# warwick-hpsc/MG-CFD-app-plain

Measured on AMD Instinct MI355X. Metric: Medges/s (compute_flux_edge) + MG V-cycle wall-s, higher is better.
Workload: dtype f64; 1 GPU; M6-L0-like synthetic level (67^3 jittered lattice, permuted ids): 300763 nodes / 888822 internal edges per GPU, flux + update sweep, no MG; numerics=exact (bit-identical to the reference), parallelism=1 GPU, workload_kind=level0

## Files before the change

### include/mgcfd.h

```cpp
#ifndef MGCFD_H
#define MGCFD_H

#include <stdint.h>

#ifdef __cplusplus
extern "C" {
#endif

#define MGCFD_NVAR 5
#define MGCFD_RK 3

#define MGCFD_MESH_FVCORR 0
#define MGCFD_MESH_M6_WING 2
#define MGCFD_MESH_LA_CASCADE 3
#define MGCFD_MESH_ROTOR_37 4

#define MGCFD_OK 0
#define MGCFD_ERR_ARG 1
#define MGCFD_ERR_IO 2
#define MGCFD_ERR_HIP 3
#define MGCFD_ERR_NAN 4
#define MGCFD_ERR_NEG_DENSITY 5
#define MGCFD_ERR_NEG_ENERGY 6
#define MGCFD_ERR_VALIDATION 7
// ... 52 lines not shown
int mgcfd_mesh_level(const mgcfd_mesh *m, int level, mgcfd_level_desc *out);

int mgcfd_write_array(const char *path, const double *data, int64_t nel, int ncols);
int mgcfd_identify_differences(const double *test_values, const double *master_values, int64_t nel,
                               int mesh_variant, int64_t *first_bad);

int mgcfd_create(const mgcfd_level_desc *levels, int nlevels, int mesh_variant, int device,
                 mgcfd_solver **out);
int mgcfd_create_from_mesh(const mgcfd_mesh *m, int device, mgcfd_solver **out);
int mgcfd_create_partitioned(const mgcfd_level_desc *levels, int nlevels, int mesh_variant, int device,
                             const int64_t *n_owned, mgcfd_solver **out);
int mgcfd_create_partitioned_mg(const mgcfd_level_desc *levels, int nlevels, int mesh_variant, int device,
                                const int64_t *n_owned, const int64_t *const *order_keys, mgcfd_solver **out);
int mgcfd_plan_audit(const mgcfd_level_desc *levels, int nlevels, int mesh_variant, const int64_t *n_owned,
                     const int64_t *const *order_keys, char *report, int64_t report_cap);
void mgcfd_destroy(mgcfd_solver *s);
int mgcfd_set_option(mgcfd_solver *s, int option, int value);
int mgcfd_level_has_edge_once(const mgcfd_solver *s, int level, int *yes);
int mgcfd_level_has_half_rows(const mgcfd_solver *s, int level, int *yes);
int mgcfd_level_has_order_free(const mgcfd_solver *s, int level, int *yes);
int mgcfd_level_stage_wg4(const mgcfd_solver *s, int level, int *yes);
int mgcfd_level_tiling(const mgcfd_solver *s, int level, int64_t out[10]);
int mgcfd_get_option(const mgcfd_solver *s, int option, int *value);
int mgcfd_set_stream(mgcfd_solver *s, void *hip_stream);
int mgcfd_synchronize(mgcfd_solver *s);
int mgcfd_num_levels(const mgcfd_solver *s);
int64_t mgcfd_level_nel(const mgcfd_solver *s, int level);
int64_t mgcfd_level_num_internal_edges(const mgcfd_solver *s, int level);
int mgcfd_get_far_field(const mgcfd_solver *s, double *out17);
int mgcfd_free_stream_constants(double mach, double alpha_deg, double out17[17]);
// ... 124 lines not shown
```

### mg-cfd-app-plain_amd/csrc/device_plan.hpp

```cpp
#pragma once

#include <hip/hip_runtime.h>
#include <cstdint>

#include "preprocess.hpp"

namespace mgcfd {

constexpr int kNumStateFields = 5;
static_assert(sizeof(EdgeW) == 32, "EdgeW must be 32 bytes");
static_assert(sizeof(ProlongW) == 24, "ProlongW must be 24 bytes");

constexpr int kVariantStageWg4 = 1 << 7;

struct FarField {
    double var[5];
    double fc_mx[3], fc_my[3], fc_mz[3], fc_de[3];
};

constexpr int kMaxPushPeers = 8;
struct PushPeers {
    double *base[kMaxPushPeers] = {nullptr, nullptr, nullptr, nullptr, nullptr, nullptr, nullptr, nullptr};
    int64_t stride[kMaxPushPeers] = {0, 0, 0, 0, 0, 0, 0, 0};
    int64_t first[kMaxPushPeers + 1] = {0, 0, 0, 0, 0, 0, 0, 0, 0};
    int n = 0;
};

struct PushFlags {
// ... 113 lines not shown
    double p_inf = 0.0;
    const double *ref = nullptr;
    const int32_t *slot = nullptr;
    double *table = nullptr;
    int64_t row = 0;
};

struct TailPlan {
    const int32_t *rows_main = nullptr;
    const int32_t *tile_ptr = nullptr;
    const double2 *rec = nullptr;
    const int32_t *begin = nullptr, *count = nullptr;
    double2 *flux = nullptr;
};

struct DevicePlan {
    int64_t nel = 0;
    int64_t stride = 0;
    int32_t n_slices = 0;
    int32_t *slice_row0 = nullptr, *rows_int = nullptr, *rows_bnd = nullptr, *nbr = nullptr;
    double *w = nullptr;
    int32_t n_tiles = 0;
    int32_t pad_row = 0;
    int32_t pad_chunk = 0;
    uint16_t *nbr16 = nullptr;
    int32_t *tile_halo = nullptr;
    int32_t *tile_ovf_ptr = nullptr, *tile_ovf = nullptr;
    int vin_ok = 0;
    int lds_complete = 0;
    int32_t halo_max = 0;
    int edge_once = 0;
    int32_t *te_chunk_ptr = nullptr, *te_count = nullptr;
    uint16_t *te_slots = nullptr, *gat16 = nullptr;
    double *te_w = nullptr;
    double *te_w3 = nullptr;
// ... 31 lines not shown
```

### mg-cfd-app-plain_amd/csrc/kernels.hip

```cpp
#include <hip/hip_runtime.h>
#include <algorithm>
#include <cstdlib>
#include <stdexcept>
#include <stdint.h>
#include <type_traits>

#include "device_plan.hpp"

#ifndef MGCFD_KERNEL_NS
#error "compile with -DMGCFD_KERNEL_NS=exact|fast"
#endif

namespace mgcfd {
namespace MGCFD_KERNEL_NS {

#ifdef MGCFD_PHASES
__device__ unsigned long long g_phase[4096 * 8];
__device__ unsigned long long g_phase_abs[4096 * 8];
#define PH_MARK(k) do { if (threadIdx.x == 0) { unsigned long long now_ = wall_clock64(); g_phase[(blockIdx.x & 4095) * 8 + (k)] += now_ - ph_last_; ph_last_ = now_; g_phase_abs[(blockIdx.x & 4095) * 8 + 1 + (k)] = now_; } } while (0)
#define PH_BEGIN() unsigned long long ph_last_ = wall_clock64(); if (threadIdx.x == 0) { g_phase[(blockIdx.x & 4095) * 8 + 7] += 1ull; g_phase_abs[(blockIdx.x & 4095) * 8] = ph_last_; \
        g_phase_abs[(blockIdx.x & 4095) * 8 + 7] = (static_cast<unsigned long long>(__builtin_amdgcn_s_getreg(20 | (0 << 6) | (31 << 11))) << 32) | __builtin_amdgcn_s_getreg(4 | (0 << 6) | (31 << 11)); }
#else
#define PH_MARK(k) do { } while (0)
#define PH_BEGIN() do { } while (0)
#endif

#if defined(MGCFD_EXP_FLUX_ST_NT)
#define MGCFD_ST_FLUX(p, v) __builtin_nontemporal_store((v), (p))
#elif defined(MGCFD_EXP_FLUX_ST_PLAIN)
#define MGCFD_ST_FLUX(p, v) (*(p) = (v))
#else
#define MGCFD_ST_FLUX(p, v) __hip_atomic_store((p), (v), __ATOMIC_RELAXED, __HIP_MEMORY_SCOPE_AGENT)
#endif
#if defined(MGCFD_EXP_STAGE_ST_PLAIN)
#define MGCFD_ST_STAGE(p, v) (*(p) = (v))
#elif defined(MGCFD_EXP_STAGE_ST_NT)
#define MGCFD_ST_STAGE(p, v) __builtin_nontemporal_store((v), (p))
#else
#define MGCFD_ST_STAGE(p, v) __hip_atomic_store((p), (v), __ATOMIC_RELAXED, __HIP_MEMORY_SCOPE_AGENT)
// ... 159 lines not shown

__device__ __forceinline__ double wave_sum(double v)
{
    for (int off = 32; off > 0; off >>= 1) v += __shfl_xor(v, off);
    return v;
}

__device__ __forceinline__ unsigned long long err_key(int check, int32_t original_id, int code)
{
    return (static_cast<unsigned long long>(check) << 40) | (static_cast<unsigned long long>(uint32_t(original_id)) << 8) | unsigned(code);
}

__device__ __forceinline__ unsigned xcd_contiguous_block(unsigned b, unsigned nb)
{
    const unsigned q = nb >> 3, r = nb & 7u, x = b & 7u, k = b >> 3;
    return (x < r ? x * (q + 1) : r * (q + 1) + (x - r) * q) + k;
}

}

__global__ void __launch_bounds__(kBlock)
k_init_variables(int64_t stride, FarField ff, double *__restrict__ q)
{
    const int64_t i = blockIdx.x * int64_t(kBlock) + threadIdx.x;
    if (i >= stride) return;
    store_conserved(q, stride, i, ff.var[0], ff.var[1], ff.var[2], ff.var[3], ff.var[4]);
}

__global__ void __launch_bounds__(kBlock)
k_step_factor_local(int64_t nel, int64_t stride, const double *__restrict__ q, const double *__restrict__ cbrt_vol,
                    double cfl, double *__restrict__ step_factors, double *__restrict__ partial_min,
// ... 293 lines not shown
}

struct FluxTileLds {
    double2 tile[kTileCap * kLdsRecD2];
    double s_pm[kBlock / 64];
    double s_next[2][kBlock / 64];
};
struct FluxTileLds4 {
    double2 tile[kTileCap4 * kLdsRec80D2];
    double s_pm[kBlock / 64];
    double s_next[2][kBlock / 64];
};
static_assert(sizeof(FluxTileLds4) <= 160 * 1024 / 4, "four workgroups per CU");
static_assert(kTileCap4 - kTile < kBlock, "one halo id per thread");

template <int WMODE, bool FUSE, bool ACC, int ROLE, bool TAIL, bool PUSH, bool SLIM = false, typename Lds = FluxTileLds>
__device__ __forceinline__ void
flux_tile_body(Lds &lds, const unsigned block,
               const double *__restrict__ q, const int32_t *__restrict__ tile_halo, uint32_t n_tiles, int32_t pad_row,
               int64_t stride, int64_t nel, const int32_t *__restrict__ slice_row0,
               const int32_t *__restrict__ rows_int, const int32_t *__restrict__ rows_bnd,
               const uint16_t *__restrict__ nbr16, const double *__restrict__ w,
               const int32_t *__restrict__ tile_ovf_ptr, const int32_t *__restrict__ tile_ovf, const FarField &ff,
               double *__restrict__ fluxes, int classes, const FusedStep &fs, const TailPlan &tp,
               const uint16_t *__restrict__ gat16, const int32_t *__restrict__ te_chunk_ptr, const double *__restrict__ te_w3,
               const StagePush &push ,
               const bool block_is_tile = false )
{
    constexpr bool LOADK = WMODE == 1;
    static_assert(!PUSH || FUSE, "only a fused stage sends its message");
    PH_BEGIN();
    constexpr bool IDXW = WMODE == 2;
    static_assert(!(IDXW && TAIL), "indexed weights: levels without long rows only");
    static_assert(!SLIM || (!TAIL && !IDXW && !PUSH && ROLE != 5), "80-byte records: the stages without long rows, indexed weights, message or absorbed stage");
    double2 *const tile = lds.tile;

    double min_dt = 0.0;
    constexpr int kPartPre = 6;
    double *const s_pm = lds.s_pm;
    double pmv[kPartPre];

    const int tid = threadIdx.x;
    const int lane = tid & 63;
    unsigned t = block_is_tile ? block : xcd_contiguous_block(block, n_tiles);
    if (PUSH) {
        const unsigned nb = unsigned(push.n_boundary);
        t = block < nb ? block : nb + xcd_contiguous_block(block - nb, n_tiles - nb);
    }
    if (FUSE && fs.tile_list) t = unsigned(fs.tile_list[t]);
    const int64_t base = int64_t(t) * kTile;
    const int64_t i = base + tid;
    const int32_t slice = __builtin_amdgcn_readfirstlane(static_cast<int32_t>(i >> 6));

    const int32_t *hrow = tile_halo + int64_t(t) * kHaloStride;
    const int32_t hid = hrow[tid];
    const int32_t hid2 = (!SLIM && ROLE != 5 && tid < kHaloStride - kBlock) ? hrow[kBlock + tid] : -1;
    const int32_t row0 = slice_row0[slice];
    const int32_t n_int = (classes & 1) ? (TAIL ? tp.rows_main : rows_int)[slice] : 0;
    const int32_t n_bnd = rows_bnd[slice];
    const bool has_halo = hid >= 0;
    const int64_t hnode = has_halo ? int64_t(hid) : i;
    double o0, o1, o2, o3, o4, g0, g1, g2, g3, g4;
    EdgeRow e0, e1;
    RowRef i0{}, i1{}, i2{}, i3{};
    const double *tw = nullptr;
    if (IDXW) {
        i0 = load_ref(nbr16, gat16, n_int > 0 ? row0 : pad_row, lane);
        i1 = load_ref(nbr16, gat16, n_int > 1 ? row0 + 1 : pad_row, lane);
        i2 = load_ref(nbr16, gat16, n_int > 2 ? row0 + 2 : pad_row, lane);
        i3 = load_ref(nbr16, gat16, n_int > 3 ? row0 + 3 : pad_row, lane);
        tw = te_w3 + int64_t(te_chunk_ptr[t]) * (kEdgeChunk * 3);
    }
    if (FUSE && ROLE == 5) {
#pragma unroll
// ... 229 lines not shown
            }                                                                                                     \
        } while (0)
        if (n_glob > 0) {
            const double2 *in = tp.flux + 3 * int64_t(tl_nb);
            MGCFD_ADD_ENTRIES(in, n_glob);
        }
        {
            const double2 *in = tile + 3 * (tl_nb + n_glob - last0);
            const int32_t n_lds = tl_nc - n_glob;
            MGCFD_ADD_ENTRIES(in, n_lds);
        }
#undef MGCFD_ADD_ENTRIES
    }

    if ((classes & 6) && n_bnd > 0) {
        const int32_t first_bnd = rows_int[slice];
        const FluxC fm = fm_pre;
        for (int32_t r = 0; r < n_bnd; r++) {
            const EdgeRow e = load_row<false>(nbr16, w, int64_t(row0) + first_bnd + r, lane);
            const double fx = e.fx, fy = e.fy, fz = e.fz;
            if (e.code == kT16Wall && (classes & 2)) {
                a0 += 0.0;
                a1 += fx * me.p;
                a2 += fy * me.p;
                a3 += fz * me.p;
                a4 += 0.0;
            } else if (e.code == kT16Far && (classes & 4)) {
                a0 += fx * (ff.var[1] + me.mx) + fy * (ff.var[2] + me.my) + fz * (ff.var[3] + me.mz);
                a4 += fx * (ff.fc_de[0] + fm.ex) + fy * (ff.fc_de[1] + fm.ey) + fz * (ff.fc_de[2] + fm.ez);
                a1 += fx * (ff.fc_mx[0] + fm.xx) + fy * (ff.fc_mx[1] + fm.xy) + fz * (ff.fc_mx[2] + fm.xz);
                a2 += fx * (ff.fc_my[0] + fm.xy) + fy * (ff.fc_my[1] + fm.yy) + fz * (ff.fc_my[2] + fm.yz);
                a3 += fx * (ff.fc_mz[0] + fm.xz) + fy * (ff.fc_mz[1] + fm.yz) + fz * (ff.fc_mz[2] + fm.zz);
            }
        }
// ... 9 lines not shown
    }
    double sf_next = __longlong_as_double(0x7FF0000000000000LL);
    double ss = 0.0;
    if (i < nel) {
        double sf = sfv;
        if (ROLE == 0 || ROLE == 5) {
            min_dt = s_pm[0];
            for (int wv = 1; wv < kBlock / 64; wv++) min_dt = fmin(min_dt, s_pm[wv]);
            sf = min_dt / sfv;
            fs.step_factors[i] = sf;
        }
        const double factor = sf / fs.rk_div;
        const double rho = r0 + factor * a0, mx = r1 + factor * a1, my = r2 + factor * a2, mz = r3 + factor * a3,
                     en = r4 + factor * a4;
        store_conserved(fs.q_out, stride, i, rho, mx, my, mz, en);
        if (ROLE >= 2 && ROLE <= 4) {
            const double d0 = rho - r0, d1 = mx - r1, d2 = my - r2, d3 = mz - r3, d4 = en - r4;
            if (fs.residuals) {
                MGCFD_ST_STAGE(fs.residuals + i, d0); MGCFD_ST_STAGE(fs.residuals + stride + i, d1); MGCFD_ST_STAGE(fs.residuals + 2 * stride + i, d2);
                MGCFD_ST_STAGE(fs.residuals + 3 * stride + i, d3); MGCFD_ST_STAGE(fs.residuals + 4 * stride + i, d4);
            }
            if (fs.sumsq_partial) ss = (((d0 * d0 + d1 * d1) + d2 * d2) + d3 * d3) + d4 * d4;
        }
        if (fs.check) {
            const bool finite = isfinite(rho) && isfinite(mx) && isfinite(my) && isfinite(mz) && isfinite(en);
            int code = 0;
            if (!finite) code = 1;
            else if (rho < 0.0) code = 2;
            else if (en < 0.0) code = 3;
            if (code) atomicMin(fs.err, err_key(fs.check, fs.old_of_new[i], code));
// ... 38 lines not shown
        double (*const s_next)[kBlock / 64] = lds.s_next;
        if (ROLE == 3) sf_next = wave_min(sf_next);
        if (fs.sumsq_partial) ss = wave_sum(ss);
        if ((threadIdx.x & 63) == 0) { s_next[0][threadIdx.x >> 6] = sf_next; s_next[1][threadIdx.x >> 6] = ss; }
        __syncthreads();
        if (threadIdx.x == 0) {
            double m = s_next[0][0], sum = s_next[1][0];
            for (int wv = 1; wv < kBlock / 64; wv++) { m = fmin(m, s_next[0][wv]); sum += s_next[1][wv]; }
            if (ROLE == 3) fs.next_partial_min[t] = m;
            if (fs.sumsq_partial) fs.sumsq_partial[t] = sum;
        }
    }
    PH_MARK(3);
}

template <int MINW, int WMODE, bool FUSE, bool ACC, int ROLE, bool TAIL, bool PUSH = false, bool SLIM = false>
__global__ void __launch_bounds__(kBlock, MINW)
k_flux_tile(
            const double *__restrict__ q, const int32_t *__restrict__ tile_halo, uint32_t n_tiles, int32_t pad_row,
            int64_t stride, int64_t nel, const int32_t *__restrict__ slice_row0,
            const int32_t *__restrict__ rows_int, const int32_t *__restrict__ rows_bnd,
            const uint16_t *__restrict__ nbr16, const double *__restrict__ w,
            const int32_t *__restrict__ tile_ovf_ptr, const int32_t *__restrict__ tile_ovf, FarField ff,
            double *__restrict__ fluxes, int classes, FusedStep fs, TailPlan tp,
            const uint16_t *__restrict__ gat16, const int32_t *__restrict__ te_chunk_ptr, const double *__restrict__ te_w3,
            StagePush push)
{
    __shared__ std::conditional_t<SLIM, FluxTileLds4, FluxTileLds> lds;
    flux_tile_body<WMODE, FUSE, ACC, ROLE, TAIL, PUSH, SLIM>(lds, blockIdx.x, q, tile_halo, n_tiles, pad_row, stride, nel, slice_row0, rows_int, rows_bnd, nbr16, w,
                                                       tile_ovf_ptr, tile_ovf, ff, fluxes, classes, fs, tp, gat16, te_chunk_ptr, te_w3, push);
}

struct TileEdge { uint32_t sa, sb; double fx, fy, fz, k; };
constexpr int kGatherPre = 8;

template <bool LOADK>
__device__ __forceinline__ TileEdge load_tile_edge(const uint16_t *__restrict__ te_slots, const double *__restrict__ te_w,
                                                   int64_t chunk, int tid)
{
    TileEdge e;
    e.sa = te_slots[(chunk * 2) * kEdgeChunk + tid];
    e.sb = te_slots[(chunk * 2 + 1) * kEdgeChunk + tid];
    const double *wr = te_w + chunk * (4 * kEdgeChunk) + tid;
    e.fx = wr[0]; e.fy = wr[kEdgeChunk]; e.fz = wr[2 * kEdgeChunk];
    e.k = LOADK ? wr[3 * kEdgeChunk] : 0.0;
// ... 403 lines not shown
    double min_dt = 0.0;
    if (FUSE && !SPEC && fs.partial_min) min_dt = block_min_of_partials(fs.partial_min, fs.n_partial);
    constexpr int kPartPre = 6;
    __shared__ double s_pm[kBlock / 64];
    double pmv[kPartPre];

    const int tid = threadIdx.x;
    const int lane = tid & 63;
    const unsigned t = xcd_contiguous_block(blockIdx.x, n_tiles);
    const int64_t i = int64_t(t) * kTile + tid;
    const int32_t slice = __builtin_amdgcn_readfirstlane(static_cast<int32_t>(i >> 6));

    const int32_t *hrow = tile_halo + int64_t(t) * (WIDE ? kFreeHaloStride : kHaloStride);
    const int32_t hid = hrow[tid];
    const int32_t hid2 = (WIDE || tid < kHaloStride - kBlock) ? hrow[kBlock + tid] : -1;
    const int32_t h0 = hr_row0[slice];
    const int32_t n_h = (classes & 1) ? hr_row0[slice + 1] - h0 : 0;
    const int32_t n_bnd = rows_bnd[slice];
#ifdef MGCFD_ABL_FREE_OWN_AOS
    const double2 oa_ = *reinterpret_cast<const double2 *>(q + 5 * i), ob_ = *reinterpret_cast<const double2 *>(q + 5 * i + 2);
    const double o0 = oa_.x, o1 = oa_.y, o2 = ob_.x, o3 = ob_.y, o4 = q[5 * i + 4];
#else
    const double o0 = MGCFD_LD_STATE(q + i), o1 = MGCFD_LD_STATE(q + stride + i), o2 = MGCFD_LD_STATE(q + 2 * stride + i),
                 o3 = MGCFD_LD_STATE(q + 3 * stride + i), o4 = MGCFD_LD_STATE(q + 4 * stride + i);
#endif
    EdgeRow er[kHalfMaxRows];
#ifdef MGCFD_EXP_FREE_ORDER
    constexpr int kRowsFirst = MGCFD_EXP_FREE_ORDER;
#else
    constexpr int kRowsFirst = 2;
#endif
#pragma unroll
    for (int j = 0; j < kRowsFirst; j++) er[j] = load_half_row(hr_code, hr_w, j < n_h ? h0 + j : hr_pad_row, lane);
    const int64_t hnode = hid >= 0 ? int64_t(hid) : i;
#if defined(MGCFD_ABL_FREE_HALO) && MGCFD_ABL_FREE_HALO == 1
    const double2 ga_ = *reinterpret_cast<const double2 *>(q + 5 * hnode), gb_ = *reinterpret_cast<const double2 *>(q + 5 * hnode + 2);
    const double g0 = ga_.x, g1 = ga_.y, g2 = gb_.x, g3 = gb_.y, g4 = q[5 * hnode + 4];
#elif defined(MGCFD_ABL_FREE_HALO) && MGCFD_ABL_FREE_HALO == 2
    const double2 ga_ = *reinterpret_cast<const double2 *>(q + 8 * (hnode >> 1)), gb_ = *reinterpret_cast<const double2 *>(q + 8 * (hnode >> 1) + 2);
    const double g0 = ga_.x, g1 = ga_.y, g2 = gb_.x, g3 = gb_.y, g4 = q[8 * (hnode >> 1) + 4];
// ... 1507 lines not shown
template <typename F>
static void with_bool(bool b, F &&f) { if (b) f(std::true_type{}); else f(std::false_type{}); }
template <typename F>
static void with_kind(bool fused, bool accumulate, F &&f)
{
    if (fused) f(std::true_type{}, std::false_type{});
    else if (accumulate) f(std::false_type{}, std::true_type{});
    else f(std::false_type{}, std::false_type{});
}

struct FluxLaunch {
    hipStream_t st; const DevicePlan &p; const double *q; const FarField &ff; double *fluxes; int classes; const FusedStep &fs;
    dim3 grid; int64_t nel_arg;
};

template <int WMODE, bool FUSE, bool ACC, int ROLE, bool TAIL, bool PUSH = false, bool SLIM = false>
static void launch_tile(const FluxLaunch &a, const StagePush &push = StagePush{})
{
    const DevicePlan &p = a.p;
    constexpr int MINW = SLIM ? 4 : ((TAIL && (ACC || ROLE == 5)) ? 2 : 3);
    hipLaunchKernelGGL((k_flux_tile<MINW, WMODE, FUSE, ACC, ROLE, TAIL, PUSH, SLIM>), a.grid, dim3(kBlock), 0, a.st, a.q, p.tile_halo,
                       uint32_t(a.grid.x), p.pad_row, p.stride, a.nel_arg, p.slice_row0, p.rows_int, p.rows_bnd,
                       p.nbr16, p.w, p.tile_ovf_ptr, p.tile_ovf, a.ff, a.fluxes, a.classes, a.fs, p.tail, p.gat16,
                       p.te_chunk_ptr, p.te_w3, push);
}

#ifdef MGCFD_ORDER_FREE
template <bool FUSE, bool ACC, int CAP, bool LONG, bool WIDE = false, int ROLE = -1>
static void launch_free(const FluxLaunch &a)
{
    const DevicePlan &p = a.p;
    hipLaunchKernelGGL((k_flux_free<FUSE, ACC, CAP, LONG, WIDE, ROLE>), a.grid, dim3(kBlock), 0, a.st, a.q, WIDE ? p.free_halo : p.tile_halo, uint32_t(p.n_tiles),
                       p.hr_pad_row, p.stride, p.nel, p.hr_row0, p.hr_code, p.hr_w, p.slice_row0,
                       p.rows_int, p.rows_bnd, p.nbr16, p.w, a.ff, a.fluxes, a.classes, a.fs);
}

static int free_stage_role(const FusedStep &fs, int role)
{
    if (fs.next_legacy_sf) return -1;
// ... 19 lines not shown

void launch_flux(hipStream_t st, const DevicePlan &p, const double *q, const FarField &ff, double *fluxes,
                 int classes, int accumulate, int variant, const FusedStep *fused, const StagePush *push)
{
    FusedStep fs{};
    if (fused) fs = *fused;
    const bool part = fused && fs.tile_list;
    if (part && fs.n_list <= 0) return;
    const FluxLaunch a{st, p, q, ff, fluxes, classes, fs, dim3(part ? fs.n_list : p.n_tiles), (fused && fs.nel_active > 0) ? fs.nel_active : p.nel};
    const int role = fused ? stage_role(fs) : 1;
    const bool tail = p.has_tail && (classes & 1);
    const bool loadk = (variant & 1) == 0;
    if (push && fused && part && !fs.vin_flux) {
        check_first_stage_input(role, q, fs);
        with_bool(loadk, [&](auto K) { with_bool(tail, [&](auto T) { with_constant<0, 1, 2, 3, 4>(role, [&](auto R) {
            launch_tile<decltype(K)::value ? 1 : 0, true, false, decltype(R)::value, decltype(T)::value, true>(a, *push);
        }); }); });
        return;
    }
    check_first_stage_input(role, q, fs);
    if ((variant & 4) && !fused && p.edge_flux) {
        if (classes & 1)
            hipLaunchKernelGGL(k_fission_edge_flux, dim3(grid_for(p.n_edges)), dim3(kBlock), 0, st, p.n_edges, p.n_edges_pad, p.stride, q,
                               p.fe_ab, p.fe_w, p.edge_flux);
        with_bool(accumulate != 0, [&](auto A) {
            hipLaunchKernelGGL(k_fission_node_sum<decltype(A)::value>, a.grid, dim3(kBlock), 0, st, p.nel, p.stride, p.n_edges_pad, q, p.slice_row0,
                               p.rows_int, p.rows_bnd, p.row_edge, p.nbr16, p.w, p.edge_flux, ff, fluxes, classes);
        });
        return;
    }
#ifdef MGCFD_ORDER_FREE
// ... 21 lines not shown
            hipLaunchKernelGGL((k_flux_half<decltype(F)::value, decltype(A)::value>), a.grid, dim3(kBlock), 0, st, q, p.tile_halo, uint32_t(p.n_tiles),
                               p.hr_pad_row, p.stride, p.nel, p.hr_row0, p.hr_code, p.hr_w, p.hg16, p.slice_row0,
                               p.rows_int, p.rows_bnd, p.pad_row, p.nbr16, p.w, ff, fluxes, classes, fs);
        });
        return;
    }
    if ((variant & 2) && p.edge_once && (classes & 1) && !part) {
        with_bool(loadk, [&](auto K) { with_kind(fused, accumulate, [&](auto F, auto A) {
            hipLaunchKernelGGL((k_flux_edge_once<decltype(K)::value, decltype(F)::value, decltype(A)::value>), a.grid, dim3(kBlock), 0, st, q, p.tile_halo,
                               uint32_t(p.n_tiles), p.pad_row, p.stride, p.nel, p.te_chunk_ptr, p.te_count,
                               p.pad_chunk, classes, p.slice_row0, p.rows_int, p.rows_bnd, p.nbr16, p.w, p.gat16,
                               p.te_slots, p.te_w, p.tile_ovf_ptr, p.tile_ovf, ff, fluxes, fs);
        }); });
        return;
    }
    const bool indexed = (variant & 16) && p.edge_once && p.te_w3 && !tail;
#ifndef MGCFD_ORDER_FREE
    if (fused && (variant & kVariantStageWg4) && stage_wg4_fits(p) && !indexed && role != 5) {
        with_bool(loadk, [&](auto K) { with_constant<0, 1, 2, 3, 4>(role, [&](auto R) {
            launch_tile<decltype(K)::value ? 1 : 0, true, false, decltype(R)::value, false, false, true>(a);
        }); });
        return;
    }
#endif
    with_constant<0, 1, 2>(indexed ? 2 : (loadk ? 1 : 0), [&](auto W) { with_bool(tail, [&](auto T) {
        constexpr int WMODE = decltype(W)::value;
        constexpr bool TAIL = decltype(T)::value;
        if constexpr (!(WMODE == 2 && TAIL)) {
            if (fused) with_constant<0, 1, 2, 3, 4, 5>(role, [&](auto R) { launch_tile<WMODE, true, false, decltype(R)::value, TAIL>(a); });
            else if (accumulate) launch_tile<WMODE, false, true, 1, TAIL>(a);
            else launch_tile<WMODE, false, false, 1, TAIL>(a);
        }
    }); });
}

__global__ void __launch_bounds__(kBlock)
k_stream_tiles(const double2 *__restrict__ src, double *__restrict__ dst, int64_t rd_total2, int64_t wr_total, int rd2_per_thread, int wr_per_thread)
{
    __shared__ double lds[40960 / 8 - 64];
    const int64_t r0 = int64_t(blockIdx.x) * rd2_per_thread * kBlock + threadIdx.x;
    double acc = 0.0;
    for (int k = 0; k < rd2_per_thread; k += 8) {
        double2 v[8];
#pragma unroll
// ... 241 lines not shown
```

### mg-cfd-app-plain_amd/csrc/solver.cpp

```cpp
#include <hip/hip_runtime.h>
#include <dlfcn.h>

#include <functional>
#include <future>

#include <algorithm>
#include <atomic>
#include <cmath>
#include <cstdio>
#include <cstdlib>
#include <chrono>
#include <cstring>
#include <limits>
#include <map>
#include <memory>
#include <mutex>
#include <optional>
#include <stdexcept>
#include <string>
#include <thread>
#include <vector>

#include "device_owner.hpp"
#include "kernels.hpp"
// ... 443 lines not shown
    bool stage_wg4_for(const DeviceLevel &lv) const
    {
        if (!opt_exact || !opt_stage_wg4 || !stage_wg4_fits(lv.dp)) return false;
        if (n_cus == 0) {
            use_device();
            HIP_CHECK(hipDeviceGetAttribute(&n_cus, hipDeviceAttributeMultiprocessorCount, device));
        }
        return lv.dp.n_tiles > 3 * n_cus;
    }
    void op_flux(int l, int classes)
    {
        DeviceLevel &lv = level(l);
        Timed t(this, l, MGCFD_LOOP_FLUX, (classes & 1) != 0);
        if (classes != 7) settle_fluxes(lv);
        const int accumulate = lv.fluxes_zero ? 0 : 1;
        const int variant = variant_for(lv);
        if ((variant & 4) && !lv.dp.edge_flux)
            lv.dp.edge_flux = lv.mem.alloc<double>(static_cast<size_t>(lv.dp.n_edges_pad) * 5 + 8);
        k().flux(stream, lv.dp, lv.q, ff, lv.fluxes, classes, accumulate, variant, nullptr, nullptr);
        if ((classes & 1) && jst_on(l)) {
            const JstStep a = jst_step(lv);
            k().jst_sensor(stream, lv.dp, a);
            k().jst_dissipation(stream, lv.dp, a);
        }
        if (dual_time()) lv.flux_in = lv.q;
        lv.fluxes_zero = false;
        lv.fluxes_stale = false;
        if (classes & 1) lv.iters[MGCFD_LOOP_FLUX] += lv.info.n_internal;
    }
    void op_fused_stage(int l, int j, const double *in, double *out, const StageArgs &a = StageArgs{})
    {
// ... 393 lines not shown
        st.alloc(lv.residuals, sizeof(double) * (static_cast<size_t>(stride) * 5));
        st.alloc(lv.step_factors, sizeof(double) * (static_cast<size_t>(stride)));
        st.alloc(lv.sf_alt, sizeof(double) * (static_cast<size_t>(stride)));
        st.alloc(lv.min_dt, sizeof(double) * (1));
        st.upload(lv.partial_min, std::vector<double>(static_cast<size_t>((nel + 255) / 256), std::numeric_limits<double>::infinity()));
        st.alloc(lv.tile_sumsq, sizeof(double) * (static_cast<size_t>((nel + 255) / 256)));
        st.alloc(lv.sumsq, sizeof(double) * (1));
        lv.n_partials = static_cast<int>(std::min<int64_t>(1024, (nel * 5 + 255) / 256));
        st.alloc(lv.partials, sizeof(double) * (static_cast<size_t>(lv.n_partials)));
        lv.dp.nel = nel;
        lv.dp.stride = stride;
        lv.dp.n_slices = P.n_slices;
        st.upload(lv.dp.slice_row0, P.slice_row0);
        st.upload(lv.dp.rows_int, P.rows_int);
        st.upload(lv.dp.rows_bnd, P.rows_bnd);
        {
            std::vector<double> ws(P.w.size() * 4 + 2 * 4 * kSlice, 0.0);
            for (size_t e = 0; e < P.w.size(); e++) {
                const size_t row = e / kSlice, lane = e % kSlice;
                ws[(row * 4 + 0) * kSlice + lane] = P.w[e].x;
                ws[(row * 4 + 1) * kSlice + lane] = P.w[e].y;
                ws[(row * 4 + 2) * kSlice + lane] = P.w[e].z;
                ws[(row * 4 + 3) * kSlice + lane] = P.w[e].k;
            }
            st.upload(lv.dp.w, std::move(ws));
        }
        st.upload(lv.dp.old_of_new, P.old_of_new);
        lv.dp.n_tiles = P.n_tiles;
        lv.plan.nbr16.resize(P.nbr16.size() + 2 * kSlice, static_cast<uint16_t>(kT16Pad));
        st.upload(lv.dp.nbr16, P.nbr16);
// ... 258 lines not shown
        }
        for (int l = 0; l < nlevels; l++) {
            const std::string r = audit_level_plan(levels[l], plans[static_cast<size_t>(l)], l + 1 < nlevels ? levels[l + 1].nel : -1);
            if (!r.empty()) rep += "level " + std::to_string(l) + ":\n" + r;
            if (std::getenv("MGCFD_PLAN_DIGEST")) {
                char buf[64];
                std::snprintf(buf, sizeof(buf), "digest level %d: %016llx\n", l, (unsigned long long)plan_digest(plans[static_cast<size_t>(l)]));
                rep += buf;
            }
        }
    });
    if (rc != MGCFD_OK) return rc;
    if (report && report_cap > 0) { std::snprintf(report, static_cast<size_t>(report_cap), "%s", rep.c_str()); }
    if (!rep.empty()) { g_last_error = "plan audit: " + rep; return MGCFD_ERR_ARG; }
    return MGCFD_OK;
}

int mgcfd_create(const mgcfd_level_desc *levels, int nlevels, int mesh_variant, int device, mgcfd_solver **out)
{
    REQUIRE(out);
    return guarded([&] { *out = build_solver(levels, nlevels, mesh_variant, device).release(); });
}
int mgcfd_create_partitioned(const mgcfd_level_desc *levels, int nlevels, int mesh_variant, int device,
                             const int64_t *n_owned, mgcfd_solver **out)
{
    REQUIRE(out); REQUIRE(n_owned);
    return guarded([&] { *out = build_solver(levels, nlevels, mesh_variant, device, n_owned).release(); });
}
int mgcfd_create_partitioned_mg(const mgcfd_level_desc *levels, int nlevels, int mesh_variant, int device,
                                const int64_t *n_owned, const int64_t *const *order_keys, mgcfd_solver **out)
// ... 1089 lines not shown
        s->use_device();
        s->fold_events();
        DeviceLevel &lv = s->level(level);
        *launches = lv.flux_launches;
        *avg_seconds = lv.flux_launches ? lv.flux_time / double(lv.flux_launches) : 0.0;
    });
}

int mgcfd_bench_flux(mgcfd_solver *s, int level, int launches, double *avg_seconds)
{
    REQUIRE(s); REQUIRE(avg_seconds);
    return guarded([&] {
        s->use_device();
        DeviceLevel &lv = s->level(level);
        Event a = s->get_event(), b = s->get_event();
        const int variant = s->variant_for(lv);
        if ((variant & 4) && !lv.dp.edge_flux)
            lv.dp.edge_flux = lv.mem.alloc<double>(static_cast<size_t>(lv.dp.n_edges_pad) * 5 + 8);
        auto go = [&] {
            s->k().flux(s->stream, lv.dp, lv.q, s->ff, lv.fluxes, 7, 0, variant, nullptr, nullptr);
        };
        go();
        HIP_CHECK(hipEventRecord(a.get(), s->stream));
        for (int k = 0; k < launches; k++) go();
        HIP_CHECK(hipEventRecord(b.get(), s->stream));
        HIP_CHECK(hipStreamSynchronize(s->stream));
        float ms = 0.f;
        HIP_CHECK(hipEventElapsedTime(&ms, a.get(), b.get()));
        s->free_events.push_back(std::move(a));
        s->free_events.push_back(std::move(b));
        lv.fluxes_zero = false;
// ... 2206 lines not shown
```

### mg-cfd-app-plain_amd/mgcfd/__init__.py

```python
from . import meshgen
from .api import (EXPORTED_SYMBOLS, LIB_PATH, LOOPS, Group, MgcfdError, Mesh, Solver,
                  free_stream_constants, generated_to_levels, live_device_resources, load_coefficients, load_library, plan_audit,
                  rccl_unique_id)
```

### mg-cfd-app-plain_amd/mgcfd/api.py

```python
from __future__ import annotations

import ctypes as C
import os
import sys
from typing import List, Optional, Sequence

import numpy as np

from .meshgen import EDGE_DTYPE, LevelMesh, MultigridMesh, to_edge_arrays

PKG_DIR = os.path.dirname(os.path.abspath(__file__))
CSRC_DIR = os.path.normpath(os.path.join(PKG_DIR, "..", "csrc"))
LIB_PATH = os.environ.get("MGCFD_LIB") or os.path.join(CSRC_DIR, "libmgcfd_hip.so")

NVAR = 5
RK = 3
LOOPS = ("flux", "update", "compute_step", "time_step", "restrict", "prolong", "indirect_rw")
ARR = {"variables": 0, "old_variables": 1, "fluxes": 2, "residuals": 3, "step_factors": 4, "volumes": 5, "stage": 6,
       "time_n": 7, "time_n1": 8, "jst_laplacian": 9, "jst_sensor": 10, "jst_radius": 11,
       "fas_forcing": 12, "fas_start": 13}
OPT = {"exact": 0, "timing": 1, "indirect_rw": 2, "check_invalid": 3, "flux_variant": 4, "fuse_update": 5, "graph": 6, "rank_split": 7, "stage_wg4": 8}
ERR_NAMES = {0: "OK", 1: "ERR_ARG", 2: "ERR_IO", 3: "ERR_HIP", 4: "ERR_NAN", 5: "ERR_NEG_DENSITY",
             6: "ERR_NEG_ENERGY", 7: "ERR_VALIDATION"}

# ... 27 lines not shown

_SIGNATURES = [
    ("mgcfd_last_error", C.c_char_p, []),
    ("mgcfd_abi_version", C.c_int, []),
    ("mgcfd_mesh_load", C.c_int, [C.c_char_p, C.c_char_p, C.c_int, C.POINTER(_vp)]),
    ("mgcfd_mesh_load_ex", C.c_int, [C.c_char_p, C.c_char_p, C.c_int, C.c_int, C.POINTER(_vp)]),
    ("mgcfd_mesh_free", None, [_vp]),
    ("mgcfd_mesh_num_levels", C.c_int, [_vp]),
    ("mgcfd_mesh_variant", C.c_int, [_vp]),
    ("mgcfd_mesh_size", C.c_int, [_vp]),
    ("mgcfd_mesh_level", C.c_int, [_vp, C.c_int, C.POINTER(LevelDesc)]),
    ("mgcfd_write_array", C.c_int, [C.c_char_p, _vp, _i64, C.c_int]),
    ("mgcfd_identify_differences", C.c_int, [_vp, _vp, _i64, C.c_int, C.POINTER(_i64)]),
    ("mgcfd_create", C.c_int, [C.POINTER(LevelDesc), C.c_int, C.c_int, C.c_int, C.POINTER(_vp)]),
    ("mgcfd_plan_audit", C.c_int, [C.POINTER(LevelDesc), C.c_int, C.c_int, C.POINTER(_i64), C.POINTER(C.POINTER(_i64)), C.c_char_p, _i64]),
    ("mgcfd_create_partitioned_mg", C.c_int, [C.POINTER(LevelDesc), C.c_int, C.c_int, C.c_int, C.POINTER(_i64),
                                                 C.POINTER(C.POINTER(_i64)), C.POINTER(_vp)]),
    ("mgcfd_create_from_mesh", C.c_int, [_vp, C.c_int, C.POINTER(_vp)]),
    ("mgcfd_create_partitioned", C.c_int, [C.POINTER(LevelDesc), C.c_int, C.c_int, C.c_int, C.POINTER(_i64), C.POINTER(_vp)]),
    ("mgcfd_halo_plan", C.c_int, [_vp, C.c_int, _i64, _vp, C.POINTER(C.c_int)]),
    ("mgcfd_halo_pack", C.c_int, [_vp, C.c_int, C.c_int, C.c_int, _vp]),
    ("mgcfd_halo_unpack", C.c_int, [_vp, C.c_int, C.c_int, C.c_int, _vp]),
    ("mgcfd_destroy", None, [_vp]),
    ("mgcfd_live_device_resources", C.c_int, [C.POINTER(_i64)]),
    ("mgcfd_set_option", C.c_int, [_vp, C.c_int, C.c_int]),
    ("mgcfd_level_has_edge_once", C.c_int, [_vp, C.c_int, C.POINTER(C.c_int)]),
    ("mgcfd_level_has_half_rows", C.c_int, [_vp, C.c_int, C.POINTER(C.c_int)]),
    ("mgcfd_pending_invalid_state", C.c_int, [_vp, C.POINTER(C.c_int64)]),
    ("mgcfd_level_has_order_free", C.c_int, [_vp, C.c_int, C.POINTER(C.c_int)]),
    ("mgcfd_level_stage_wg4", C.c_int, [_vp, C.c_int, C.POINTER(C.c_int)]),
# ... 222 lines not shown
    lib = load_library()
    descs, keep = _level_descs(levels)
    owned = None if n_owned is None else (_i64 * len(levels))(*[int(v) for v in n_owned])
    kp = None
    if order_keys is not None:
        keys = [None if k is None else np.ascontiguousarray(k, dtype=np.int64) for k in order_keys]
        keep += keys
        kp = (C.POINTER(_i64) * len(levels))(*[C.cast(_ptr(k), C.POINTER(_i64)) if k is not None else C.POINTER(_i64)() for k in keys])
    buf = C.create_string_buffer(1 << 16)
    rc = lib.mgcfd_plan_audit(descs, len(levels), mesh_variant, owned, kp, buf, len(buf))
    if rc not in (0, 1):
        _check(lib, rc)
    return buf.value.decode()


def load_coefficients(ff17, loads, ref_area: float = 1.0, ref_length: float = 1.0) -> np.ndarray:
    lib = load_library()
    ff = np.ascontiguousarray(ff17, dtype=np.float64).reshape(17)
    rows = np.ascontiguousarray(loads, dtype=np.float64)
    flat = rows.reshape(-1, 6)
    out = np.zeros_like(flat)
    for k in range(len(flat)):
        row = np.ascontiguousarray(flat[k])
        res = np.zeros(6)
        _check(lib, lib.mgcfd_load_coefficients(_ptr(ff), _ptr(row), float(ref_area), float(ref_length), _ptr(res)))
        out[k] = res
    return out.reshape(rows.shape)


def free_stream_constants(mach: float, alpha_deg: float) -> np.ndarray:
# ... 554 lines not shown
```

Baseline: 52520 Medges/s.

## Pack per-slice metadata into one 16-byte record and slim kernel arguments

Replaces the three separate per-slice arrays (row0, interior/main rows, boundary rows) with a packed 16-byte SliceRec that the flux tile kernel reads in a single int4 load, and precomputes the first boundary row. Kernel arguments for fused state, tail plan, indexed weights and push are wrapped in compile-time optional holders so unused template instantiations do not carry them. It also enables the stage-wg4 (four workgroups per CU) path for unfused flux launches and adds a LIST template flag so the tile-list indirection is compiled out of whole-level launches. It adds a host-side slice table export API. The risk is more template instantiations and new launch-time checks.

Measured after the change: 52640 Medges/s, median of 5. Within noise of the previous version (+0.2%).

```diff
diff --git a/include/mgcfd.h b/include/mgcfd.h
--- a/include/mgcfd.h
+++ b/include/mgcfd.h
@@ -90,6 +90,8 @@
                                 const int64_t *n_owned, const int64_t *const *order_keys, mgcfd_solver **out);
 int mgcfd_plan_audit(const mgcfd_level_desc *levels, int nlevels, int mesh_variant, const int64_t *n_owned,
                      const int64_t *const *order_keys, char *report, int64_t report_cap);
+int mgcfd_plan_slice_table(const mgcfd_level_desc *level, int mesh_variant, int64_t n_owned, int64_t cap_slices,
+                           int32_t *table, int32_t *vectors, int64_t *n_slices, int *has_tail);
 void mgcfd_destroy(mgcfd_solver *s);
 int mgcfd_set_option(mgcfd_solver *s, int option, int value);
 int mgcfd_level_has_edge_once(const mgcfd_solver *s, int level, int *yes);
diff --git a/mg-cfd-app-plain_amd/csrc/device_plan.hpp b/mg-cfd-app-plain_amd/csrc/device_plan.hpp
--- a/mg-cfd-app-plain_amd/csrc/device_plan.hpp
+++ b/mg-cfd-app-plain_amd/csrc/device_plan.hpp
@@ -2,6 +2,7 @@
 
 #include <hip/hip_runtime.h>
 #include <cstdint>
+#include <vector>
 
 #include "preprocess.hpp"
 
@@ -12,6 +13,7 @@
 static_assert(sizeof(ProlongW) == 24, "ProlongW must be 24 bytes");
 
 constexpr int kVariantStageWg4 = 1 << 7;
+constexpr int kVariantWholeLevel = 1 << 8;
 
 struct FarField {
     double var[5];
@@ -155,11 +157,24 @@
     double2 *flux = nullptr;
 };
 
+struct SliceRec { int32_t row0, n_loop, n_bnd, first_bnd; };
+static_assert(sizeof(SliceRec) == 16, "SliceRec must be 16 bytes");
+
+inline std::vector<SliceRec> pack_slice_table(const LevelPlan &P)
+{
+    std::vector<SliceRec> t(static_cast<size_t>(P.n_slices) + 1);
+    for (size_t s = 0; s < static_cast<size_t>(P.n_slices); s++)
+        t[s] = SliceRec{P.slice_row0[s], P.has_tail ? P.rows_main[s] : P.rows_int[s], P.rows_bnd[s], P.slice_row0[s] + P.rows_int[s]};
+    t.back() = SliceRec{P.slice_row0.back(), 0, 0, P.slice_row0.back()};
+    return t;
+}
+
 struct DevicePlan {
     int64_t nel = 0;
     int64_t stride = 0;
     int32_t n_slices = 0;
     int32_t *slice_row0 = nullptr, *rows_int = nullptr, *rows_bnd = nullptr, *nbr = nullptr;
+    SliceRec *slices = nullptr;
     double *w = nullptr;
     int32_t n_tiles = 0;
     int32_t pad_row = 0;
diff --git a/mg-cfd-app-plain_amd/csrc/kernels.hip b/mg-cfd-app-plain_amd/csrc/kernels.hip
--- a/mg-cfd-app-plain_amd/csrc/kernels.hip
+++ b/mg-cfd-app-plain_amd/csrc/kernels.hip
@@ -17,12 +17,14 @@
 #ifdef MGCFD_PHASES
 __device__ unsigned long long g_phase[4096 * 8];
 __device__ unsigned long long g_phase_abs[4096 * 8];
-#define PH_MARK(k) do { if (threadIdx.x == 0) { unsigned long long now_ = wall_clock64(); g_phase[(blockIdx.x & 4095) * 8 + (k)] += now_ - ph_last_; ph_last_ = now_; g_phase_abs[(blockIdx.x & 4095) * 8 + 1 + (k)] = now_; } } while (0)
-#define PH_BEGIN() unsigned long long ph_last_ = wall_clock64(); if (threadIdx.x == 0) { g_phase[(blockIdx.x & 4095) * 8 + 7] += 1ull; g_phase_abs[(blockIdx.x & 4095) * 8] = ph_last_; \
-        g_phase_abs[(blockIdx.x & 4095) * 8 + 7] = (static_cast<unsigned long long>(__builtin_amdgcn_s_getreg(20 | (0 << 6) | (31 << 11))) << 32) | __builtin_amdgcn_s_getreg(4 | (0 << 6) | (31 << 11)); }
+#define PH_MARK(k) do { if (threadIdx.x == 0) { unsigned long long now_ = wall_clock64(); g_phase[ph_slot_ * 8 + (k)] += now_ - ph_last_; ph_last_ = now_; if ((k) < 6) g_phase_abs[ph_slot_ * 8 + 1 + (k)] = now_; } } while (0)
+#define PH_BEGIN_AT(first) const unsigned ph_slot_ = (blockIdx.x + (first)) & 4095u; unsigned long long ph_last_ = wall_clock64(); if (threadIdx.x == 0) { g_phase[ph_slot_ * 8 + 7] += 1ull; g_phase_abs[ph_slot_ * 8] = ph_last_; \
+        g_phase_abs[ph_slot_ * 8 + 7] = (static_cast<unsigned long long>(__builtin_amdgcn_s_getreg(20 | (0 << 6) | (31 << 11))) << 32) | __builtin_amdgcn_s_getreg(4 | (0 << 6) | (31 << 11)); }
+#define PH_BEGIN() PH_BEGIN_AT(0u)
 #else
 #define PH_MARK(k) do { } while (0)
 #define PH_BEGIN() do { } while (0)
+#define PH_BEGIN_AT(first) do { } while (0)
 #endif
 
 #if defined(MGCFD_EXP_FLUX_ST_NT)
@@ -212,7 +214,7 @@
 __device__ __forceinline__ unsigned xcd_contiguous_block(unsigned b, unsigned nb)
 {
     const unsigned q = nb >> 3, r = nb & 7u, x = b & 7u, k = b >> 3;
-    return (x < r ? x * (q + 1) : r * (q + 1) + (x - r) * q) + k;
+    return x * q + min(x, r) + k;
 }
 
 }
@@ -536,12 +538,11 @@
 static_assert(sizeof(FluxTileLds4) <= 160 * 1024 / 4, "four workgroups per CU");
 static_assert(kTileCap4 - kTile < kBlock, "one halo id per thread");
 
-template <int WMODE, bool FUSE, bool ACC, int ROLE, bool TAIL, bool PUSH, bool SLIM = false, typename Lds = FluxTileLds>
+template <int WMODE, bool FUSE, bool ACC, int ROLE, bool TAIL, bool PUSH, bool SLIM = false, bool LIST = false, typename Lds = FluxTileLds>
 __device__ __forceinline__ void
 flux_tile_body(Lds &lds, const unsigned block,
                const double *__restrict__ q, const int32_t *__restrict__ tile_halo, uint32_t n_tiles, int32_t pad_row,
-               int64_t stride, int64_t nel, const int32_t *__restrict__ slice_row0,
-               const int32_t *__restrict__ rows_int, const int32_t *__restrict__ rows_bnd,
+               int64_t stride, int64_t nel, const SliceRec *__restrict__ slices,
                const uint16_t *__restrict__ nbr16, const double *__restrict__ w,
                const int32_t *__restrict__ tile_ovf_ptr, const int32_t *__restrict__ tile_ovf, const FarField &ff,
                double *__restrict__ fluxes, int classes, const FusedStep &fs, const TailPlan &tp,
@@ -551,7 +552,8 @@
 {
     constexpr bool LOADK = WMODE == 1;
     static_assert(!PUSH || FUSE, "only a fused stage sends its message");
-    PH_BEGIN();
+    static_assert(!LIST || FUSE, "only a fused stage runs over a tile list");
+    PH_BEGIN_AT(FUSE ? (ROLE == 0 ? 0u : (ROLE == 1 ? 1280u : 2560u)) : 0u);
     constexpr bool IDXW = WMODE == 2;
     static_assert(!(IDXW && TAIL), "indexed weights: levels without long rows only");
     static_assert(!SLIM || (!TAIL && !IDXW && !PUSH && ROLE != 5), "80-byte records: the stages without long rows, indexed weights, message or absorbed stage");
@@ -569,7 +571,8 @@
         const unsigned nb = unsigned(push.n_boundary);
         t = block < nb ? block : nb + xcd_contiguous_block(block - nb, n_tiles - nb);
     }
-    if (FUSE && fs.tile_list) t = unsigned(fs.tile_list[t]);
+    if (LIST) t = unsigned(fs.tile_list[t]);
+    PH_MARK(4);
     const int64_t base = int64_t(t) * kTile;
     const int64_t i = base + tid;
     const int32_t slice = __builtin_amdgcn_readfirstlane(static_cast<int32_t>(i >> 6));
@@ -577,9 +580,10 @@
     const int32_t *hrow = tile_halo + int64_t(t) * kHaloStride;
     const int32_t hid = hrow[tid];
     const int32_t hid2 = (!SLIM && ROLE != 5 && tid < kHaloStride - kBlock) ? hrow[kBlock + tid] : -1;
-    const int32_t row0 = slice_row0[slice];
-    const int32_t n_int = (classes & 1) ? (TAIL ? tp.rows_main : rows_int)[slice] : 0;
-    const int32_t n_bnd = rows_bnd[slice];
+    const int4 srec = *reinterpret_cast<const int4 *>(slices + slice);
+    const int32_t row0 = srec.x;
+    const int32_t n_int = (classes & 1) ? srec.y : 0;
+    const int32_t n_bnd = srec.z;
     const bool has_halo = hid >= 0;
     const int64_t hnode = has_halo ? int64_t(hid) : i;
     double o0, o1, o2, o3, o4, g0, g1, g2, g3, g4;
@@ -839,10 +843,9 @@
     }
 
     if ((classes & 6) && n_bnd > 0) {
-        const int32_t first_bnd = rows_int[slice];
         const FluxC fm = fm_pre;
         for (int32_t r = 0; r < n_bnd; r++) {
-            const EdgeRow e = load_row<false>(nbr16, w, int64_t(row0) + first_bnd + r, lane);
+            const EdgeRow e = load_row<false>(nbr16, w, int64_t(srec.w) + r, lane);
             const double fx = e.fx, fy = e.fy, fz = e.fz;
             if (e.code == kT16Wall && (classes & 2)) {
                 a0 += 0.0;
@@ -882,6 +885,7 @@
         const double rho = r0 + factor * a0, mx = r1 + factor * a1, my = r2 + factor * a2, mz = r3 + factor * a3,
                      en = r4 + factor * a4;
         store_conserved(fs.q_out, stride, i, rho, mx, my, mz, en);
+        PH_MARK(5);
         if (ROLE >= 2 && ROLE <= 4) {
             const double d0 = rho - r0, d1 = mx - r1, d2 = my - r2, d3 = mz - r3, d4 = en - r4;
             if (fs.residuals) {
@@ -950,21 +954,32 @@
     PH_MARK(3);
 }
 
-template <int MINW, int WMODE, bool FUSE, bool ACC, int ROLE, bool TAIL, bool PUSH = false, bool SLIM = false>
+template <typename T, bool ON> struct OptArg {
+    T v;
+    OptArg(const T &x) : v(x) {}
+    __device__ const T &get() const { return v; }
+};
+template <typename T> struct OptArg<T, false> {
+    OptArg(const T &) {}
+    __device__ T get() const { return T{}; }
+};
+struct IndexedW { const uint16_t *gat16 = nullptr; const int32_t *te_chunk_ptr = nullptr; const double *te_w3 = nullptr; };
+
+template <int MINW, int WMODE, bool FUSE, bool ACC, int ROLE, bool TAIL, bool PUSH = false, bool SLIM = false, bool LIST = false>
 __global__ void __launch_bounds__(kBlock, MINW)
 k_flux_tile(
-            const double *__restrict__ q, const int32_t *__restrict__ tile_halo, uint32_t n_tiles, int32_t pad_row,
-            int64_t stride, int64_t nel, const int32_t *__restrict__ slice_row0,
-            const int32_t *__restrict__ rows_int, const int32_t *__restrict__ rows_bnd,
+            const double *__restrict__ q, const int32_t *__restrict__ tile_halo, uint32_t n_tiles, int classes,
+            int64_t stride, const SliceRec *__restrict__ slices,
             const uint16_t *__restrict__ nbr16, const double *__restrict__ w,
+            int32_t pad_row, int64_t nel,
             const int32_t *__restrict__ tile_ovf_ptr, const int32_t *__restrict__ tile_ovf, FarField ff,
-            double *__restrict__ fluxes, int classes, FusedStep fs, TailPlan tp,
-            const uint16_t *__restrict__ gat16, const int32_t *__restrict__ te_chunk_ptr, const double *__restrict__ te_w3,
-            StagePush push)
+            double *__restrict__ fluxes, OptArg<FusedStep, FUSE> fs, OptArg<TailPlan, TAIL> tp,
+            OptArg<IndexedW, WMODE == 2> iw, OptArg<StagePush, PUSH> push)
 {
     __shared__ std::conditional_t<SLIM, FluxTileLds4, FluxTileLds> lds;
-    flux_tile_body<WMODE, FUSE, ACC, ROLE, TAIL, PUSH, SLIM>(lds, blockIdx.x, q, tile_halo, n_tiles, pad_row, stride, nel, slice_row0, rows_int, rows_bnd, nbr16, w,
-                                                       tile_ovf_ptr, tile_ovf, ff, fluxes, classes, fs, tp, gat16, te_chunk_ptr, te_w3, push);
+    const IndexedW ix = iw.get();
+    flux_tile_body<WMODE, FUSE, ACC, ROLE, TAIL, PUSH, SLIM, LIST>(lds, blockIdx.x, q, tile_halo, n_tiles, pad_row, stride, nel, slices, nbr16, w,
+                                                             tile_ovf_ptr, tile_ovf, ff, fluxes, classes, fs.get(), tp.get(), ix.gat16, ix.te_chunk_ptr, ix.te_w3, push.get());
 }
 
 struct TileEdge { uint32_t sa, sb; double fx, fy, fz, k; };
@@ -1398,9 +1413,6 @@
     const int32_t *hrow = tile_halo + int64_t(t) * (WIDE ? kFreeHaloStride : kHaloStride);
     const int32_t hid = hrow[tid];
     const int32_t hid2 = (WIDE || tid < kHaloStride - kBlock) ? hrow[kBlock + tid] : -1;
-    const int32_t h0 = hr_row0[slice];
-    const int32_t n_h = (classes & 1) ? hr_row0[slice + 1] - h0 : 0;
-    const int32_t n_bnd = rows_bnd[slice];
 #ifdef MGCFD_ABL_FREE_OWN_AOS
     const double2 oa_ = *reinterpret_cast<const double2 *>(q + 5 * i), ob_ = *reinterpret_cast<const double2 *>(q + 5 * i + 2);
     const double o0 = oa_.x, o1 = oa_.y, o2 = ob_.x, o3 = ob_.y, o4 = q[5 * i + 4];
@@ -1408,6 +1420,9 @@
     const double o0 = MGCFD_LD_STATE(q + i), o1 = MGCFD_LD_STATE(q + stride + i), o2 = MGCFD_LD_STATE(q + 2 * stride + i),
                  o3 = MGCFD_LD_STATE(q + 3 * stride + i), o4 = MGCFD_LD_STATE(q + 4 * stride + i);
 #endif
+    const int32_t h0 = hr_row0[slice], h1 = hr_row0[slice + 1];
+    const int32_t n_h = (classes & 1) ? h1 - h0 : 0;
+    const int32_t n_bnd = rows_bnd[slice];
     EdgeRow er[kHalfMaxRows];
 #ifdef MGCFD_EXP_FREE_ORDER
     constexpr int kRowsFirst = MGCFD_EXP_FREE_ORDER;
@@ -2945,15 +2960,17 @@
     dim3 grid; int64_t nel_arg;
 };
 
-template <int WMODE, bool FUSE, bool ACC, int ROLE, bool TAIL, bool PUSH = false, bool SLIM = false>
+template <int WMODE, bool FUSE, bool ACC, int ROLE, bool TAIL, bool PUSH = false, bool SLIM = false, bool LIST = false>
 static void launch_tile(const FluxLaunch &a, const StagePush &push = StagePush{})
 {
     const DevicePlan &p = a.p;
+    if (!LIST && a.fs.tile_list) throw std::logic_error("a tile list given to a whole-level stage launch");
+    if (LIST && !a.fs.tile_list) throw std::logic_error("a listed stage launch without its tile list");
     constexpr int MINW = SLIM ? 4 : ((TAIL && (ACC || ROLE == 5)) ? 2 : 3);
-    hipLaunchKernelGGL((k_flux_tile<MINW, WMODE, FUSE, ACC, ROLE, TAIL, PUSH, SLIM>), a.grid, dim3(kBlock), 0, a.st, a.q, p.tile_halo,
-                       uint32_t(a.grid.x), p.pad_row, p.stride, a.nel_arg, p.slice_row0, p.rows_int, p.rows_bnd,
-                       p.nbr16, p.w, p.tile_ovf_ptr, p.tile_ovf, a.ff, a.fluxes, a.classes, a.fs, p.tail, p.gat16,
-                       p.te_chunk_ptr, p.te_w3, push);
+    hipLaunchKernelGGL((k_flux_tile<MINW, WMODE, FUSE, ACC, ROLE, TAIL, PUSH, SLIM, LIST>), a.grid, dim3(kBlock), 0, a.st, a.q, p.tile_halo,
+                       uint32_t(a.grid.x), a.classes, p.stride, p.slices, p.nbr16, p.w, p.pad_row, a.nel_arg,
+                       p.tile_ovf_ptr, p.tile_ovf, a.ff, a.fluxes, OptArg<FusedStep, FUSE>(a.fs), OptArg<TailPlan, TAIL>(p.tail),
+                       OptArg<IndexedW, WMODE == 2>(IndexedW{p.gat16, p.te_chunk_ptr, p.te_w3}), OptArg<StagePush, PUSH>(push));
 }
 
 #ifdef MGCFD_ORDER_FREE
@@ -3003,7 +3020,7 @@
     if (push && fused && part && !fs.vin_flux) {
         check_first_stage_input(role, q, fs);
         with_bool(loadk, [&](auto K) { with_bool(tail, [&](auto T) { with_constant<0, 1, 2, 3, 4>(role, [&](auto R) {
-            launch_tile<decltype(K)::value ? 1 : 0, true, false, decltype(R)::value, decltype(T)::value, true>(a, *push);
+            launch_tile<decltype(K)::value ? 1 : 0, true, false, decltype(R)::value, decltype(T)::value, true, false, true>(a, *push);
         }); }); });
         return;
     }
@@ -3055,12 +3072,19 @@
         }); });
         return;
     }
-    const bool indexed = (variant & 16) && p.edge_once && p.te_w3 && !tail;
+    const bool indexed = (variant & 16) && p.edge_once && p.te_w3 && !tail && !part;
+    const bool listed = part && !(variant & kVariantWholeLevel);
 #ifndef MGCFD_ORDER_FREE
+    if (!fused && (variant & kVariantStageWg4) && stage_wg4_fits(p) && !indexed) {
+        with_bool(loadk, [&](auto K) { with_bool(accumulate != 0, [&](auto A) {
+            launch_tile<decltype(K)::value ? 1 : 0, false, decltype(A)::value, 1, false, false, true>(a);
+        }); });
+        return;
+    }
     if (fused && (variant & kVariantStageWg4) && stage_wg4_fits(p) && !indexed && role != 5) {
-        with_bool(loadk, [&](auto K) { with_constant<0, 1, 2, 3, 4>(role, [&](auto R) {
-            launch_tile<decltype(K)::value ? 1 : 0, true, false, decltype(R)::value, false, false, true>(a);
-        }); });
+        with_bool(loadk, [&](auto K) { with_bool(listed, [&](auto L) { with_constant<0, 1, 2, 3, 4>(role, [&](auto R) {
+            launch_tile<decltype(K)::value ? 1 : 0, true, false, decltype(R)::value, false, false, true, decltype(L)::value>(a);
+        }); }); });
         return;
     }
 #endif
@@ -3068,7 +3092,10 @@
         constexpr int WMODE = decltype(W)::value;
         constexpr bool TAIL = decltype(T)::value;
         if constexpr (!(WMODE == 2 && TAIL)) {
-            if (fused) with_constant<0, 1, 2, 3, 4, 5>(role, [&](auto R) { launch_tile<WMODE, true, false, decltype(R)::value, TAIL>(a); });
+            if (fused) with_bool(listed, [&](auto L) { with_constant<0, 1, 2, 3, 4, 5>(role, [&](auto R) {
+                constexpr bool LIST = decltype(L)::value;
+                if constexpr (!(WMODE == 2 && LIST)) launch_tile<WMODE, true, false, decltype(R)::value, TAIL, false, false, LIST>(a);
+            }); });
             else if (accumulate) launch_tile<WMODE, false, true, 1, TAIL>(a);
             else launch_tile<WMODE, false, false, 1, TAIL>(a);
         }
diff --git a/mg-cfd-app-plain_amd/csrc/solver.cpp b/mg-cfd-app-plain_amd/csrc/solver.cpp
--- a/mg-cfd-app-plain_amd/csrc/solver.cpp
+++ b/mg-cfd-app-plain_amd/csrc/solver.cpp
@@ -481,7 +481,7 @@
         Timed t(this, l, MGCFD_LOOP_FLUX, (classes & 1) != 0);
         if (classes != 7) settle_fluxes(lv);
         const int accumulate = lv.fluxes_zero ? 0 : 1;
-        const int variant = variant_for(lv);
+        const int variant = variant_for(lv) | (stage_wg4_for(lv) ? kVariantStageWg4 : 0);
         if ((variant & 4) && !lv.dp.edge_flux)
             lv.dp.edge_flux = lv.mem.alloc<double>(static_cast<size_t>(lv.dp.n_edges_pad) * 5 + 8);
         k().flux(stream, lv.dp, lv.q, ff, lv.fluxes, classes, accumulate, variant, nullptr, nullptr);
@@ -905,6 +905,7 @@
         st.upload(lv.dp.slice_row0, P.slice_row0);
         st.upload(lv.dp.rows_int, P.rows_int);
         st.upload(lv.dp.rows_bnd, P.rows_bnd);
+        st.upload(lv.dp.slices, pack_slice_table(P));
         {
             std::vector<double> ws(P.w.size() * 4 + 2 * 4 * kSlice, 0.0);
             for (size_t e = 0; e < P.w.size(); e++) {
@@ -1193,6 +1194,34 @@
     if (report && report_cap > 0) { std::snprintf(report, static_cast<size_t>(report_cap), "%s", rep.c_str()); }
     if (!rep.empty()) { g_last_error = "plan audit: " + rep; return MGCFD_ERR_ARG; }
     return MGCFD_OK;
+}
+
+int mgcfd_plan_slice_table(const mgcfd_level_desc *level, int mesh_variant, int64_t n_owned, int64_t cap_slices,
+                           int32_t *table, int32_t *vectors, int64_t *n_slices, int *has_tail)
+{
+    REQUIRE(level); REQUIRE(n_slices);
+    return guarded([&] {
+        const mgcfd_level_desc &d = *level;
+        if (!d.volumes || !d.edges) throw std::invalid_argument("level is missing volumes/edges");
+        std::vector<mgcfd_edge> edges(d.edges, d.edges + d.n_edges);
+        adjust_and_dampen(d, mesh_variant, edges);
+        PlanOptions popt;
+        if (n_owned >= 0 && n_owned < d.nel) popt.n_owned = n_owned;
+        LevelPlan P;
+        build_level_plan(d, edges, popt, P);
+        *n_slices = P.n_slices;
+        if (has_tail) *has_tail = P.has_tail ? 1 : 0;
+        if (!table || !vectors || cap_slices <= P.n_slices) return;
+        const std::vector<SliceRec> t = pack_slice_table(P);
+        const size_t n = static_cast<size_t>(P.n_slices) + 1;
+        for (size_t s = 0; s < n; s++) {
+            table[4 * s] = t[s].row0; table[4 * s + 1] = t[s].n_loop; table[4 * s + 2] = t[s].n_bnd; table[4 * s + 3] = t[s].first_bnd;
+            vectors[s] = P.slice_row0[s];
+            vectors[n + s] = s + 1 < n ? P.rows_int[s] : -1;
+            vectors[2 * n + s] = s + 1 < n ? P.rows_main[s] : -1;
+            vectors[3 * n + s] = s + 1 < n ? P.rows_bnd[s] : -1;
+        }
+    });
 }
 
 int mgcfd_create(const mgcfd_level_desc *levels, int nlevels, int mesh_variant, int device, mgcfd_solver **out)
@@ -2312,7 +2341,7 @@
         s->use_device();
         DeviceLevel &lv = s->level(level);
         Event a = s->get_event(), b = s->get_event();
-        const int variant = s->variant_for(lv);
+        const int variant = s->variant_for(lv) | (s->stage_wg4_for(lv) ? kVariantStageWg4 : 0);
         if ((variant & 4) && !lv.dp.edge_flux)
             lv.dp.edge_flux = lv.mem.alloc<double>(static_cast<size_t>(lv.dp.n_edges_pad) * 5 + 8);
         auto go = [&] {
diff --git a/mg-cfd-app-plain_amd/mgcfd/__init__.py b/mg-cfd-app-plain_amd/mgcfd/__init__.py
--- a/mg-cfd-app-plain_amd/mgcfd/__init__.py
+++ b/mg-cfd-app-plain_amd/mgcfd/__init__.py
@@ -1,4 +1,4 @@
 from . import meshgen
 from .api import (EXPORTED_SYMBOLS, LIB_PATH, LOOPS, Group, MgcfdError, Mesh, Solver,
-                  free_stream_constants, generated_to_levels, live_device_resources, load_coefficients, load_library, plan_audit,
+                  free_stream_constants, generated_to_levels, live_device_resources, load_coefficients, load_library, plan_audit, plan_slice_table,
                   rccl_unique_id)
diff --git a/mg-cfd-app-plain_amd/mgcfd/api.py b/mg-cfd-app-plain_amd/mgcfd/api.py
--- a/mg-cfd-app-plain_amd/mgcfd/api.py
+++ b/mg-cfd-app-plain_amd/mgcfd/api.py
@@ -65,6 +65,8 @@
     ("mgcfd_identify_differences", C.c_int, [_vp, _vp, _i64, C.c_int, C.POINTER(_i64)]),
     ("mgcfd_create", C.c_int, [C.POINTER(LevelDesc), C.c_int, C.c_int, C.c_int, C.POINTER(_vp)]),
     ("mgcfd_plan_audit", C.c_int, [C.POINTER(LevelDesc), C.c_int, C.c_int, C.POINTER(_i64), C.POINTER(C.POINTER(_i64)), C.c_char_p, _i64]),
+    ("mgcfd_plan_slice_table", C.c_int, [C.POINTER(LevelDesc), C.c_int, _i64, _i64, C.POINTER(C.c_int32), C.POINTER(C.c_int32),
+                                            C.POINTER(_i64), C.POINTER(C.c_int)]),
     ("mgcfd_create_partitioned_mg", C.c_int, [C.POINTER(LevelDesc), C.c_int, C.c_int, C.c_int, C.POINTER(_i64),
                                                  C.POINTER(C.POINTER(_i64)), C.POINTER(_vp)]),
     ("mgcfd_create_from_mesh", C.c_int, [_vp, C.c_int, C.POINTER(_vp)]),
@@ -317,6 +319,22 @@
     return buf.value.decode()
 
 
+def plan_slice_table(level: dict, mesh_variant: int, n_owned: int = -1) -> dict:
+    lib = load_library()
+    descs, keep = _level_descs([level])
+    n, tail = _i64(0), C.c_int(0)
+    _check(lib, lib.mgcfd_plan_slice_table(descs, mesh_variant, int(n_owned), 0, None, None, C.byref(n), C.byref(tail)))
+    rows = n.value + 1
+    table = np.zeros((rows, 4), dtype=np.int32)
+    vec = np.zeros((4, rows), dtype=np.int32)
+    i32p = C.POINTER(C.c_int32)
+    _check(lib, lib.mgcfd_plan_slice_table(descs, mesh_variant, int(n_owned), rows, table.ctypes.data_as(i32p), vec.ctypes.data_as(i32p),
+                                           C.byref(n), C.byref(tail)))
+    del keep
+    return {"table": table, "slice_row0": vec[0].copy(), "rows_int": vec[1, :-1].copy(), "rows_main": vec[2, :-1].copy(),
+            "rows_bnd": vec[3, :-1].copy(), "has_tail": bool(tail.value)}
+
+
 def load_coefficients(ff17, loads, ref_area: float = 1.0, ref_length: float = 1.0) -> np.ndarray:
     lib = load_library()
     ff = np.ascontiguousarray(ff17, dtype=np.float64).reshape(17)
```
